# StanfordMSL/RATiLQR.jl

Hardware: AMD Instinct MI355X
Metric: iLEQG solves/sec (N=50, n=12, m=4) at CE batch=1024 (higher is better)
Workload: dtype f64

## Files before the change

ratilqr.jl_amd/csrc/driver.cpp:

```cpp
#include <hip/hip_runtime.h>

#include <algorithm>
#include <cctype>
#include <cmath>
#include <cstdint>
#include <cstdio>
#include <cstdlib>
#include <cstring>
#include <functional>
#include <initializer_list>
#include <string>
#include <vector>

#include "../../include/ratilqr.h"
#include "kernels.h"
#include "layout.h"
#include "wide.h"
#include "ce_device.h"
#include "policy_mc.h"
#include "rare_event.h"
#include "source_args.h"
#include "source_model.h"

static thread_local std::string g_err;
// ... 14 lines not shown
    int device = 0;
    hipStream_t stream = nullptr;
    hipStream_t stream2 = nullptr;
    hipEvent_t ev_a = nullptr, ev_b = nullptr;
    bool dual_forced = false;
    bool dual = false;
    bool speculate = false;
    bool fused = true;
    bool fused_req = true, rounds_only = false;
    int block_req = -1;
    bool wdiag = true;
    bool materialize = false;
    std::vector<double> x0_host, u0_host;
    int fused_occ2 = -1;
    bool fused_dual = true;
    int block_mode = -1;
    int block_max_b = 512;
    int n_cu = 256;
    long long *d_xw = nullptr;
    int *d_duo_count = nullptr;
    bool lq_replay = true;
    bool lq_replay_last = true;
    bool lq_replay_stack = true;
    RecDev rec = {};
    size_t rec_cap = 0;
    unsigned xepoch = 0;
    int *d_census = nullptr;
    bool block_shape = true;
    bool block_helpers = true;
    bool block_acl = false;
    int path_fixed = RAT_PATH_AUTO;
    bool fly_multi = true;
    bool fly = true;
    rat_ileqg_opts opts;
    OptsDev opd;
    int Bmax = 0, E = 1;
    bool have_problem = false;
    int n = 0, m = 0, N = 0;
    ProblemDev pb;
    bool wide = false;
    WideProblemDev wpb;
    double *w_xs = nullptr, *w_us = nullptr, *w_L = nullptr, *w_dl = nullptr;
    double *w_gq = nullptr, *w_gr = nullptr, *w_gc = nullptr;
    int *w_nom = nullptr, *w_hn = nullptr;
    std::vector<void *> pb_allocs, st_allocs;
    std::vector<double> hW;
// ... 183 lines not shown
    {"ce_device", [](rat_handle h, int64_t v) { h->ce_device = (v != 0); }, [](rat_handle h) -> int64_t { return h->ce_device; }},
    {"pets_device", [](rat_handle h, int64_t v) { h->pets_device = (v != 0); }, [](rat_handle h) -> int64_t { return h->pets_device; }},
    {"psweep", [](rat_handle h, int64_t v) { h->psweep = (v < 2) ? 0 : (int)std::min<int64_t>(v, 4); }, [](rat_handle h) -> int64_t { return h->psweep; }},
    {"psw_hop", [](rat_handle h, int64_t v) { h->psw_hop = (int)std::max<int64_t>(1, v); }, [](rat_handle h) -> int64_t { return h->psw_hop; }},
    {"psw_hop_e", [](rat_handle h, int64_t v) { h->psw_hop_e = (int)std::max<int64_t>(1, v); }, [](rat_handle h) -> int64_t { return h->psw_hop_e; }},
    {"spec_force", [](rat_handle h, int64_t v) { h->spec_force = (v != 0); }, [](rat_handle h) -> int64_t { return h->spec_force; }},
    {"spec_width", [](rat_handle, int64_t) {}, [](rat_handle h) -> int64_t { return h->E; }},
    {"block_psw", [](rat_handle h, int64_t v) { h->block_psw = (v != 0); }, [](rat_handle h) -> int64_t { return h->block_psw; }},
    {"psw_duo", [](rat_handle h, int64_t v) { h->psw_duo = (v != 0); }, [](rat_handle h) -> int64_t { return h->psw_duo; }},
    {"psw_prl", [](rat_handle h, int64_t v) { h->psw_prl = (v != 0); }, [](rat_handle h) -> int64_t { return h->psw_prl; }},
    {"prl_elem", [](rat_handle h, int64_t v) { h->prl_elem = (int)std::max<int64_t>(1, v); }, [](rat_handle h) -> int64_t { return h->prl_elem; }},
    {"prl_hop", [](rat_handle h, int64_t v) { h->prl_hop = (int)std::max<int64_t>(0, v); }, [](rat_handle h) -> int64_t { return h->prl_hop; }},
    {"prl_epi", [](rat_handle h, int64_t v) { h->prl_epi = (int)std::max<int64_t>(0, v); }, [](rat_handle h) -> int64_t { return h->prl_epi; }},
    {"prl_cuts", [](rat_handle, int64_t) {}, [](rat_handle h) -> int64_t { return h->prl_last; }},
    {"psw_duo_count", [](rat_handle h, int64_t) { if (h->d_duo_count) { (void)hipStreamSynchronize(h->stream); (void)hipMemset(h->d_duo_count, 0, sizeof(int)); } },
     [](rat_handle h) -> int64_t { int c = 0; if (h->d_duo_count) { (void)hipStreamSynchronize(h->stream); (void)hipMemcpy(&c, h->d_duo_count, sizeof(int), hipMemcpyDeviceToHost); } return c; }},
    {"lq_replay", [](rat_handle h, int64_t v) { h->lq_replay = (v != 0); }, [](rat_handle h) -> int64_t { return h->lq_replay; }},
    {"lq_replay_count", [](rat_handle h, int64_t) { if (h->rec.count) { (void)hipStreamSynchronize(h->stream); (void)hipMemset(h->rec.count, 0, sizeof(int)); } },
     [](rat_handle h) -> int64_t { int c = 0; if (h->rec.count) { (void)hipStreamSynchronize(h->stream); (void)hipMemcpy(&c, h->rec.count, sizeof(int), hipMemcpyDeviceToHost); } return c; }},
    {"lq_replay_last", [](rat_handle h, int64_t v) { h->lq_replay_last = (v != 0); }, [](rat_handle h) -> int64_t { return h->lq_replay_last; }},
    {"lq_replay_last_count", [](rat_handle h, int64_t) { if (h->rec.count) { (void)hipStreamSynchronize(h->stream); (void)hipMemset(h->rec.count + 1, 0, sizeof(int)); } },
     [](rat_handle h) -> int64_t { int c = 0; if (h->rec.count) { (void)hipStreamSynchronize(h->stream); (void)hipMemcpy(&c, h->rec.count + 1, sizeof(int), hipMemcpyDeviceToHost); } return c; }},
    {"lq_replay_stack", [](rat_handle h, int64_t v) { h->lq_replay_stack = (v != 0); }, [](rat_handle h) -> int64_t { return h->lq_replay_stack; }},
    {"psw_acl", [](rat_handle h, int64_t v) { h->psw_acl = (v != 0); }, [](rat_handle h) -> int64_t { return h->psw_acl; }},
    {"psw_comp", [](rat_handle h, int64_t v) { h->psw_comp = (int)std::max<int64_t>(100, v); }, [](rat_handle h) -> int64_t { return h->psw_comp; }},
    {"src_tpw", [](rat_handle h, int64_t v) { h->src_tpw = (v >= 64) ? 64 : (v >= 32 ? 32 : 16); }, [](rat_handle h) -> int64_t { return h->src_tpw; }},
    {"src_pets_tpw", [](rat_handle h, int64_t v) { h->src_pets_tpw = (v >= 64) ? 64 : (v >= 32 ? 32 : 16); }, [](rat_handle h) -> int64_t { return h->src_pets_tpw; }},
    {"mc_cost_K", [](rat_handle, int64_t) {}, [](rat_handle h) -> int64_t { return h->mc_cost_K; }},
    {"src_mc_tpw", [](rat_handle h, int64_t v) { h->src_mc_tpw = (v >= 64) ? 64 : (v >= 32 ? 32 : 16); }, [](rat_handle h) -> int64_t { return h->src_mc_tpw; }},
    {"tail_dense", [](rat_handle h, int64_t v) { h->tail_dense = (v != 0); }, [](rat_handle h) -> int64_t { return h->tail_dense; }},
    {"src_un_loads", [](rat_handle, int64_t) {}, [](rat_handle h) -> int64_t { return h->src_un_loads; }},
};
static void finish_switches(rat_handle h) {
    h->E = (h->spec_force || h->E_req < 1) ? std::max(h->E_req, 1) : 1;
    if (!h->dual_forced) h->dual = h->E > 1;
    h->fused = h->fused_req && !(h->speculate || h->dual || h->E != 1);
    h->block_mode = h->rounds_only ? 0 : h->block_req;
}
static void debug_from_env(rat_handle h) {
    for (const DebugSwitch &sw : debug_switches) {
        std::string name = "RATILQR_";
        for (const char *c = sw.key; *c; ++c) name += (char)toupper((unsigned char)*c);
        if (const char *e = getenv(name.c_str())) {
            char *end = nullptr;
            const long long v = strtoll(e, &end, 10);
            if (end != e) sw.set(h, (int64_t)v);
// ... 960 lines not shown
    if (path == PATH_ROUNDS) launch_init_state(st, h->opd, theta_dev, h->stream);
    RolloutArgs ra; ra.st = st; ra.pb = h->pb; ra.op = h->opd; ra.dump = h->d_dump; ra.mode = 0; ra.x0 = h->d_x0; ra.u0 = h->d_u0; ra.notile = 0; ra.multi = 0;
    if (path != PATH_ROUNDS) {
        FusedArgs fa;
        fa.sw = sweep_args(h, st, 0);
        fa.sw.prune = (h->prune && st.E > 1) ? 1 : 0;
        fa.ro = ra;
        fa.max_rounds = (int)std::min<int64_t>(((int64_t)h->opd.iter_max + 1) * 4002, 2000000000);
        fa.dual = h->fused_dual ? 1 : 0;
        fa.occ2 = (path == PATH_FUSED && h->fused_dual &&
                   (h->fused_occ2 > 0 ? B >= h->fused_occ2 : (h->fused_occ2 < 0 && h->pb.model == 1 && !h->materialize && B > 4 * (int64_t)h->n_cu))) ? 1 : 0;
        fa.mat = h->materialize ? 1 : 0;
        if (path == PATH_FUSED && h->lq_replay && fa.dual && !fa.occ2 && !fa.mat && h->pb.model == 1 && h->pb.kappa == 0.0 && h->pb.W_diag &&
            !h->pb.W_tv && !h->pb.cost_tv && st.N <= ROLLIN_NST) {
            const size_t need = (size_t)B * st.N * REC_STEP;
            if (need > h->rec_cap) {
                if (h->rec.m) { HIPCHK(hipStreamSynchronize(h->stream)); HIPCHK(hipFree(h->rec.m)); h->rec.m = nullptr; h->rec_cap = 0; }
                HIPCHK(hipMalloc((void **)&h->rec.m, need * sizeof(double)));
                h->rec_cap = need;
            }
            fa.sw.rec = h->rec;
            fa.sw.rec.last = h->lq_replay_last ? 1 : 0;
            fa.sw.rec.stack = h->lq_replay_stack ? 1 : 0;
        }
        fa.theta_in = theta_dev;
        fa.out_value = out.value; fa.out_status = out.status; fa.out_iters = out.iters; fa.out_ls = out.ls;
        fa.out_cost = out.cost; fa.kl_bound = out.kl_bound;
        fa.init_x = fa.init_u = fa.init_t = nullptr;
        fa.census = (h->block_shape && h->E == 1 && B <= 2 * h->n_cu) ? h->d_census : nullptr;
        fa.helpers = (fa.census && B <= h->n_cu && h->block_helpers) ? 1 : 0;
        fa.acl = h->block_acl ? 1 : 0;
        const bool psw = path == PATH_BLOCK && h->block_psw && fa.helpers && !h->materialize && solve_block_psw_supported(fa);
        fa.duo_stride = 0; fa.xepoch = 0; fa.xw = nullptr; fa.duo_count = nullptr;
        if (psw && h->psw_duo && 2 * ((B + 7) & ~7) <= h->n_cu) {
            fa.duo_stride = (B + 7) & ~7; fa.xepoch = ++h->xepoch; fa.xw = h->d_xw; fa.duo_count = h->d_duo_count;
        }
        const bool own_init = psw && h->init_lazy && !h->init_traj_valid && h->init_batches == 0;
        if (h->init_share && h->pb.model == 1 && st.N <= ROLLIN_NST && !own_init) {
            ensure_init_traj(h, ra, theta_dev);
            fa.init_x = h->d_init_x; fa.init_u = h->d_init_u; fa.init_t = h->d_init_t;
        }
        h->init_batches++;
        fa.prl = 0;
        h->prl_last = 0;
        if (psw) {
            fa.acl = (h->psw_acl || h->block_acl) ? 1 : 0;
// ... 2994 lines not shown
```

ratilqr.jl_amd/csrc/kernels.h:

```cpp
#pragma once
#include <hip/hip_runtime.h>

#include "layout.h"

#ifndef RAT_ROLLOUT_MFMA4
#define RAT_ROLLOUT_MFMA4 1
#endif

#define REC_STEP 256
struct RecDev {
    double *m;
    double *mu;
    double *rprod;
    int *rexp;
    int *gen;
    int *lgen;
    int *count;
    int last;
    int stack;
};

struct SweepArgs {
    StateDev st;
    ProblemDev pb;
    OptsDev op;
    int mode;
    int k_first;
    const double *dl_in;
    double mu_op;
    double *op_out;
    double *dump;
    int fly;
    int prune;
    RecDev rec;
};

#define PSW_MAXP 8
struct PswCuts { int P; int cut[PSW_MAXP + 2]; };

#define PRL_WAVES 4
struct PrlCuts { int cut[PRL_WAVES + 1]; };

// ... 106 lines not shown
```

ratilqr.jl_amd/csrc/kernels.hip:

```cpp
#include <hip/hip_runtime.h>
#include <math.h>

#include "layout.h"
#include "kernels.h"

#include "device_utils.h"
#include "rat_normal.h"
#include "rat_philox.h"
#include "rat_pow.h"
#include "sweep_dual.h"

#define PART_SWEEP 1
#define PART_ROLL 2
#define PART_FUSED 4
#define PART_BLOCK2 8
#define PART_BLOCK3 16
#define PART_BLOCK5 32
#define PART_BLOCK8 64
#define PART_MISC 128
#define PART_PSW 256
#define PART_BPSW 512
#define PART_BPSW1 1024
#ifndef RAT_PART
#define RAT_PART 2047
// ... 2160 lines not shown
__device__ __forceinline__ const FusedArgs &phase_args(const FusedArgs &fa) {
    if (!LOCAL) return fa;
    auto kp = (const __attribute__((address_space(4))) FusedArgs *)__builtin_amdgcn_kernarg_segment_ptr();
    asm volatile("" : "+s"(kp));
    return *(const FusedArgs *)kp;
}
template <bool LOCAL>
__device__ __forceinline__ RolloutArgs rollout_view(const FusedArgs &pa, const int mode) {
    RolloutArgs ra;
    if (!LOCAL) { ra = pa.ro; ra.mode = mode; return ra; }
    ra.st = pa.sw.st; ra.pb = pa.sw.pb; ra.op = pa.sw.op;
    ra.mode = mode; ra.x0 = pa.ro.x0; ra.u0 = pa.ro.u0; ra.dump = pa.ro.dump; ra.notile = pa.ro.notile; ra.multi = pa.ro.multi;
    return ra;
}

template <int MODEL, bool CTV, int WM, bool DUALF, bool STG, bool OCC2 = false, bool MAT = false, bool RPL = false>
__global__ __launch_bounds__(64, OCC2 ? 2 : 1) void solve_fused_kernel(FusedArgs fa) {
    const int b = blockIdx.x;
    const StateDev &st = fa.sw.st;
#ifdef RAT_DIAG_PHASES
    const unsigned long long dg_t0 = __builtin_readcyclecounter();
    int dg_pi = 0;
#endif
    __shared__ double wls[DUALF ? WLS_DUAL : WLS_SWEEP];
    __shared__ double shxu[16];
    __shared__ double stg[STG ? STG_DOUBLES : 1];
    constexpr int FLYF = (MODEL == 1 && ((DUALF && STG && !OCC2) || (OCC2 && !DUALF && !STG)) && !MAT) ? (CTV ? 2 : 1) : 0;
    constexpr bool NT = FLYF != 0;
    constexpr bool PL = (MODEL == 1);
    constexpr bool RM4 = RAT_ROLLOUT_MFMA4 && MODEL == 1 && STG && !OCC2;
    if (threadIdx.x == 0) {
        const FusedArgs &pa = phase_args<PL>(fa);
        init_state_body(pa.sw.st, pa.sw.op, pa.theta_in, b);
        if (RPL) { pa.sw.rec.gen[b] = 0; pa.sw.rec.lgen[2 * b] = 0; pa.sw.rec.lgen[2 * b + 1] = 0; }
    }
    PHASE_FENCE();
    {
        const FusedArgs &pi = phase_args<PL>(fa);
        if (NT && pi.init_x) {
            copy_initial(pi.sw.st, pi.init_x, pi.init_u, pi.init_t, b);
        } else {
            const RolloutArgs ra = rollout_view<PL>(pi, 0);
            rollin_body<MODEL, 0, CTV, STG, true, OCC2 ? OCC2_PREFETCH : ROLLIN_PREFETCH, NT>(ra, b, shxu, stg);
        }
        PHASE_MARK();
        PHASE_FENCE();
        PHASE_MARK();
        if (DUALF) {
            SweepArgs sa = phase_args<PL>(fa).sw; sa.mode = 6;
            sweep_dual_body<WM, false, FLYF, RPL>(sa, b, wls);
            PHASE_MARK();
            PHASE_FENCE();
            if (threadIdx.x == 0) commit_init_body(phase_args<PL>(fa).sw.st, b);
            PHASE_FENCE();
            PHASE_MARK();
        } else {
            SweepArgs sa = phase_args<PL>(fa).sw; sa.mode = 2;
            sweep_body<false, false, WM, false, OCC2 ? OCC2_SWZ : 0, FLYF>(sa, b, wls);
            PHASE_MARK();
            PHASE_FENCE();
            PHASE_MARK();
        }
    }
    for (int guard = 0; guard < fa.max_rounds; ++guard) {
        const int v_stat = __atomic_load_n(&st.status[b], __ATOMIC_RELAXED), v_act = __atomic_load_n(&st.ls_active[b], __ATOMIC_RELAXED);
        if (__builtin_amdgcn_readfirstlane(v_stat) != ST_RUNNING) break;
        if (!__builtin_amdgcn_readfirstlane(v_act)) {
            SweepArgs sa = phase_args<PL>(fa).sw; sa.mode = 0;
            sweep_body<true, false, WM, false, OCC2 ? OCC2_SWZ : 0, FLYF, false, RPL>(sa, b, wls);
            PHASE_MARK();
            PHASE_FENCE();
            PHASE_MARK();
            continue;
        }
        {
            const RolloutArgs ra = rollout_view<PL>(phase_args<PL>(fa), 1);
            rollin_body<MODEL, 1, CTV, STG, true, OCC2 ? OCC2_PREFETCH : ROLLIN_PREFETCH, NT, RM4>(ra, b, shxu, stg);
            PHASE_MARK();
            PHASE_FENCE();
            PHASE_MARK();
            bool pair = DUALF;
            if (DUALF) {
                const FusedArgs &pe = phase_args<PL>(fa);
                const double v_dc = *(const volatile double *)&pe.sw.st.d_c[b], v_mu = *(const volatile double *)&pe.sw.st.mu[b];
                const int v_it = __atomic_load_n(&pe.sw.st.iter[b], __ATOMIC_RELAXED);
                const double dc = readlane_f64(v_dc, 0), mu = readlane_f64(v_mu, 0);
                const bool ends = (pe.sw.op.d > dc && mu <= pe.sw.op.mu_min) || __builtin_amdgcn_readfirstlane(v_it) == pe.sw.op.iter_max;
                pair = !ends;
            }
            if (pair) {
                SweepArgs sa = phase_args<PL>(fa).sw; sa.mode = 7;
                if (!(RPL && replay_dual_body(sa, b, wls))) sweep_dual_body<WM, true, FLYF, RPL>(sa, b, wls);
            } else {
                SweepArgs sa = phase_args<PL>(fa).sw; sa.mode = 1;
                if (!(RPL && replay_eval_body(sa, b, wls))) sweep_body<false, false, WM, true, OCC2 ? OCC2_SWZ : 0, FLYF>(sa, b, wls);
            }
            PHASE_MARK();
            PHASE_FENCE();
            if (threadIdx.x == 0) { const FusedArgs &pa = phase_args<PL>(fa); ls_select_body(pa.sw.st, pa.sw.op, b, nullptr); }
            PHASE_FENCE();
            PHASE_MARK();
        }
    }
    PHASE_FENCE();
    if (threadIdx.x == 0) {
        const FusedArgs &pa = phase_args<PL>(fa);
        gather_body(pa.sw.st, b, pa.out_value, pa.out_status, pa.out_iters, pa.out_ls, pa.out_cost, pa.kl_bound);
    }
}


#if RAT_PART & PART_FUSED
void launch_solve_fused(const FusedArgs &fa, hipStream_t s) {
    const int B = fa.sw.st.B;
    if (B <= 0) return;
// ... 1158 lines not shown
```

ratilqr.jl_amd/csrc/layout.h:

```cpp
#pragma once

#define RAT_NP 12
#define RAT_MP 4
#define RAT_PD 16
#define RAT_AUG 12

#define TS_C34 256
#define TS_R5  352
#define TS_QR  400
#define TS_q   416
#define TS_PAD 418
#define TSTRIDE 420
#define TS_INFO 417
#define TT_Q   0
#define TT_QV  144
#define TT_q   156
#define TTERM  158
#define TT_INFO 157

#define TS_LIVE(l) (((l) & 15) < 12)
#define TS_CL(l) (((l) >> 4) * 12 + ((l) & 15))
#define TS_REG(R, l) ((R) < 2 ? 2 * (l) + (R) : (R) == 2 ? 128 + 2 * (l) : (R) == 6 ? 129 + 2 * (l) : \
                      (R) < 5 ? (TS_LIVE(l) ? TS_C34 + 2 * TS_CL(l) + ((R) - 3) : TS_PAD + ((R) - 3)) : \
                                (TS_LIVE(l) ? TS_R5 + TS_CL(l) : TS_PAD))
#define TS_ZPOS(i, c) TS_REG(((i) * 16 + (c)) >> 6, ((i) * 16 + (c)) & 63)
#define TS_CPOS(i, c) TS_REG(3 + (((i) * 16 + (c)) >> 6), ((i) * 16 + (c)) & 63)

#define XSTR 12
#define USTR 4
#define LSTR 48

#define DUMP_S   0
#define DUMP_SV  144
#define DUMP_s   156
#define DUMP_g   157
#define DUMP_G   161
#define DUMP_H   209
#define DUMP_STRIDE 225

#define WLS_SWEEP 232
#define WLS_DUAL  400
#define ROLLIN_NST 52
#define STG_CL ((ROLLIN_NST * LSTR + 63) / 64)
#define STG_CX (((ROLLIN_NST + 1) * XSTR + 63) / 64)
#define STG_CU ((ROLLIN_NST * USTR + 63) / 64)
#define STG_DOUBLES ((STG_CL + STG_CX + 2 * STG_CU) * 64)
#define STG_PAD (STG_CL * 64)

#define ST_RUNNING (-1)
#define CTR_RING 8

struct ProblemDev {
    int model, n, m, N, cost_tv, W_tv;
    int W_diag;
    const double *Zt;
    const double *Ctab;
    const double *lin;
    const double *q0;
    const double *Qf;
    const double *qvf;
    double q0f, kappa;
    double pl_a, pl_b, pl_p, pl_pu, pl_cx, pl_cu, pl_h;
    const double *Winv;
    const double *Wp;
    const double *epiv;
    const double *logdetW;
    const double *Wdg;
};

// ... 33 lines not shown
```

ratilqr.jl_amd/csrc/sweep_dual.h:

```cpp
#pragma once
#include "device_utils.h"
#include "kernels.h"
#include "layout.h"

struct FlyCtx {
    double zt[3], dg[3];
    d4 cc;
    double mq, kappa;
    const double *xh;
    const double *ctab;
};
__device__ __forceinline__ void fly_init(FlyCtx &fc, const ProblemDev &pb, const double *xh, int l, int g, int j, bool tv) {
    fc.mq = (j < 12) ? 1.0 : 0.0;
    fc.kappa = pb.kappa;
    fc.xh = xh;
    fc.ctab = pb.Ctab;
#pragma unroll
    for (int r = 0; r < 3; ++r) { fc.zt[r] = pb.Zt[64 * r + l]; fc.dg[r] = (j == 4 * r + g) ? 1.0 : 0.0; }
    fc.cc = (d4){0, 0, 0, 0};
    if (!tv) {
#pragma unroll
        for (int r = 0; r < 3; ++r) fc.cc[r] = pb.Ctab[64 * r + l] * fc.mq;
        fc.cc[3] = pb.Ctab[192 + l];
    }
// ... 23 lines not shown
__device__ __forceinline__ void dload(DTile &tr, const double *__restrict__ tp, int lx, int l, int j,
                                      const double *__restrict__ Lp, double mL, int g, const FlyCtx *fc = nullptr, int t = 0) {
    if (FLY) {
        tr.xj = fc->xh[(long)t * XSTR + ((j < 12) ? j : 11)];
        if (FLY == 2) {
            const double *__restrict__ C = fc->ctab + (long)t * 256;
#pragma unroll
            for (int r = 0; r < 4; ++r) tr.c[r] = C[64 * r + l];
        }
    } else {
        const double2 *__restrict__ t2 = reinterpret_cast<const double2 *>(tp);
        const int c34 = TS_REG(3, l), r5 = TS_REG(5, l);
        const double2 w0 = t2[l], w1 = t2[64 + l], w2 = *reinterpret_cast<const double2 *>(tp + c34);
        tr.z[0] = w0.x; tr.z[1] = w0.y; tr.z[2] = w1.x; tr.z[3] = 0.0;
        tr.c[0] = w2.x; tr.c[1] = w2.y; tr.c[2] = tp[r5];
        tr.c[3] = w1.y;
    }
    tr.x = tp[TS_QR + lx];
    const int jc = (j < 12) ? j : 11;
    tr.la = HASL ? Lp[g * 12 + jc] * mL : 0.0;
}

template <int WM, bool HASL, int FLY = 0, bool REC = false>
__device__ __forceinline__ void sweep_dual_body(const SweepArgs &a, const int b, double *const wls) {
    int lane_ = threadIdx.x & 63;
    asm volatile("" : "+v"(lane_));
    const int l_ = lane_, g_ = l_ >> 4, j_ = l_ & 15;
    const int l = l_, g = g_, j = j_;
    const StateDev &st = a.st;
    const ProblemDev &pb = a.pb;
    [[maybe_unused]] const int dgs = 20 + 4 * (a.mode - 6);
    BODY_MARK(a.dump, dgs + 0);
    int slot, cidx = -1;
    const int v_act = st.ls_active[b], v_flag = st.flag_c[b * st.E], v_nom = st.slot_nom[b], v_stat = st.status[b], v_sel = st.lsel[b];
    const int s_act = wave_uniform(v_act), s_flag = wave_uniform(v_flag), s_nom = wave_uniform(v_nom), s_stat = wave_uniform(v_stat), sel = wave_uniform(v_sel);
    const double theta = st.theta[b], muB = st.mu[b];
    if (a.mode == 7) {
        if (!s_act) return;
        cidx = b * st.E;
        if (s_flag == 2) return;
        slot = cand_slot(b, 0, s_nom, st.E);
    } else {
        if (s_stat != ST_RUNNING) return;
        slot = b * (st.E + 1) + s_nom;
    }
    const double muA = (a.mode == 6) ? 0.0 : muB;
    const int N = st.N;
// ... 44 lines not shown
    const double coef = (theta != 0.0) ? -1.0 / (2.0 * theta) : 0.0;

    d4 vA, vB;
    {
        const double *__restrict__ tt = tile0 + (long)N * TSTRIDE;
#pragma unroll
        for (int r = 0; r < 3; ++r) {
            const int i = 4 * r + g;
            const double te = tt[(j < 12) ? TT_Q + i * 12 + j : TT_QV + i];
            vA[r] = (j <= 12) ? te : 0.0;
        }
        const double t3 = tt[(j < 12) ? TT_QV + j : TT_q];
        vA[3] = (g == 0 && j <= 12) ? (j < 12 ? t3 : 2.0 * t3) : 0.0;
        vB = vA;
    }
#ifdef RAT_DIAG_PHASES
    if (a.mode == 7) { asm volatile("s_waitcnt vmcnt(0)" ::: "memory"); BODY_MARK(a.dump, 29); }
#endif
    double raccA = 0.0, raccB = 0.0, rprodA = 1.0, rprodB = 1.0;
    int rexpA = 0, rexpB = 0;
    int failA = 0, deadB = 0;
    [[maybe_unused]] double *const recp = REC ? a.rec.m + (long)b * N * REC_STEP + 4 * l : nullptr;
    [[maybe_unused]] double rchk = 0.0;

    DIAG_DECL
    auto step = [&](const int t, const DTile &cur) -> int {
        int l = l_, g = g_, j = j_;
        asm volatile("" : "+v"(l), "+v"(g), "+v"(j));
        DIAG_START();
        if (WM == 1) {
#pragma unroll
            for (int r = 0; r < 3; ++r) { winv[r] = pb.Winv[(long)t * 192 + 64 * r + l]; wp[r] = pb.Wp[(long)t * 192 + 64 * r + l]; }
            { const double *ept = pb.epiv + (long)t * 16; epall = ((((ept[0] * ept[2]) * ept[4]) * ept[6]) * ept[8]) * ept[10]; }
        }
        d4 cz, ccs;
        if (!FLY) { cz = cur.z; ccs = cur.c; }
        else {
#pragma unroll
            for (int r = 0; r < 3; ++r) cz[r] = fx_diag(fc.zt[r], fc.dg[r], fc.kappa, cur.xj);
            cz[3] = 0.0;
            if (FLY == 2) { ccs[0] = cur.c[0] * fc.mq; ccs[1] = cur.c[1] * fc.mq; ccs[2] = cur.c[2] * fc.mq; ccs[3] = cur.c[3]; }
            else ccs = fc.cc;
        }
        d4 xzA, xzB;
        if (WM != 2) {
            xzA = mm3(vA, cz, (d4){0, 0, 0, 0});
// ... 68 lines not shown
        const double fvA = tmA[3] + cur.x, fvB = tmB[3] + cur.x;
        exA[g * 16 + j] = ghA; exB[g * 16 + j] = ghB;
        exA[fbo] = fvA; exB[fbo] = fvB;
        if (HASL) lbufA[l] = cur.la;
        DIAG_STAMP(3, ghB);
        WAVE_SYNC();
        const double hA0 = exA[hoff[0]], hA1 = exA[hoff[1]], hA2 = exA[hoff[2]], hA3 = exA[hoff[3]];
        const double gaA = fma(ghA, m12, exA[gaoff]);
        const double uaA = HASL ? ua_entry(hA0, hA1, hA2, hA3, lbufA[j], lbufA[16 + j], lbufA[32 + j], lbufA[48 + j], gaA) : gaA;
        const double hB0 = exB[hoff[0]], hB1 = exB[hoff[1]], hB2 = exB[hoff[2]], hB3 = exB[hoff[3]];
        const double gaB = fma(ghB, m12, exB[gaoff]);
        const double h00 = exB[12], h01 = exB[13], h02 = exB[14], h03 = exB[15];
        const double h11 = exB[16 + 13], h12 = exB[16 + 14], h13 = exB[16 + 15];
        const double h22 = exB[32 + 14], h23 = exB[32 + 15], h33 = exB[48 + 15];
        const double g0 = exB[goff[0]], g1 = exB[goff[1]], g2 = exB[goff[2]], g3 = exB[goff[3]];
        const double d0 = h00, i0 = fast_rcp(d0);
        const double l10 = h01 * i0, l20 = h02 * i0, l30 = h03 * i0;
        const double d1 = h11 - l10 * h01, i1 = fast_rcp(d1);
        const double l21 = (h12 - l20 * h01) * i1, l31 = (h13 - l30 * h01) * i1;
        const double d2 = h22 - l20 * h02 - l21 * (l21 * d1), i2 = fast_rcp(d2);
        const double l32 = (h23 - l30 * h02 - l31 * (l21 * d1)) * i2;
        const double d3 = h33 - l30 * h03 - l31 * (l31 * d1) - l32 * (l32 * d2), i3 = fast_rcp(d3);
        if (!deadB && !(d0 > 0.0 && d1 > 0.0 && d2 > 0.0 && d3 > 0.0)) deadB = 1;
        const double y0 = -g0;
        const double y1 = -g1 - l10 * y0;
        const double y2 = -g2 - l20 * y0 - l21 * y1;
        const double y3 = -g3 - l30 * y0 - l31 * y1 - l32 * y2;
        const double x3 = y3 * i3;
        const double x2 = y2 * i2 - l32 * x3;
        const double x1 = y1 * i1 - l21 * x2 - l31 * x3;
        const double x0 = y0 * i0 - l10 * x1 - l20 * x2 - l30 * x3;
        const double laB = ((x0 * em.e0[0] + x1 * em.e1[0]) + x2 * em.e0[1]) + x3 * em.e1[1];
        const double uaB = ua_entry(hB0, hB1, hB2, hB3, x0, x1, x2, x3, gaB);
        pgl[(long)t * sgl] = (j <= 12) ? laB : 0.0;
        d4 fxA, fxB;
#pragma unroll
        for (int r = 0; r < 3; ++r) { fxA[r] = fma(fA[r], m12, exA[foff[r]]); fxB[r] = fma(fB[r], m12, exB[foff[r]]); }
        const double qc = readlane_f64(cur.x, 16);
        fxA[3] = fma(fvA, mA_, (2.0 * qc + vA[3]) * mB_);
        fxB[3] = fma(fvB, mA_, (2.0 * qc + vB[3]) * mB_);
        DIAG_STAMP(4, uaB);
        d4 vnB = MFMA(laB, uaB, fxB);
        vnB = MFMA(gaB, laB, vnB);
        if (HASL) {
            d4 vnA = MFMA(cur.la, uaA, fxA);
            vA = MFMA(gaA, cur.la, vnA);
// ... 12 lines not shown
    BODY_MARK(a.dump, dgs + 1);
    for (int t = N - 1; t >= 0; t -= 2) {
        {
            const int tn = (t > 0) ? t - 1 : 0;
            dload<HASL, FLY>(rb2, tile0 + (long)tn * TSTRIDE, lx, l, j, Lb + (long)tn * LSTR, mL, g, &fc, tn);
        }
        if (step(t, ra)) break;
        if (t == 0) break;
        {
            const int tn = (t > 1) ? t - 2 : 0;
            dload<HASL, FLY>(ra, tile0 + (long)tn * TSTRIDE, lx, l, j, Lb + (long)tn * LSTR, mL, g, &fc, tn);
        }
        if (step(t - 1, rb2)) break;
    }
    BODY_MARK(a.dump, dgs + 2);
#ifdef RAT_DIAG
    if (l_ == 0 && blockIdx.x < 8 && a.dump)
        for (int q = 0; q < 6; ++q) a.dump[128 + blockIdx.x * 8 + q] = (double)dg_acc[q];
#endif
    const double totA = sweep_scalars(wave_sum(raccA), coef, rprodA, rexpA, theta != 0.0);
    (void)raccB; (void)rprodB; (void)rexpB;
    if (REC) {
        const bool bad = failA || deadB || theta == 0.0 || __ballot(!(rchk == 0.0));
        if (l == 12) rec_close(a.rec, b, sel ^ 1, bad, muB, rprodB, rexpB);
    }
    if (l == 12) {
        const double s0 = 0.5 * vA[3] + totA;
        if (a.mode == 7) {
            st.value_c[cidx] = s0;
            st.flag_c[cidx] = failA ? 1 : 0;
            if (a.prune) {
                const double cur = st.value[b], eps = st.ls_eps[b];
                const bool take = !failA && (isapprox_default(s0, cur) || s0 < cur || eps * a.op.lambda < a.op.eps_min);
                __atomic_store_n(&st.acc0[b], take ? 1 : 0, __ATOMIC_RELAXED);
            }
        } else {
            st.value[b] = failA ? INFINITY : s0;
            if (failA) st.status[b] = 1;
        }
        st.mu_spec[b] = muB;
        st.delta_spec[b] = st.delta[b];
        st.spec_st[b] = (failA || deadB == 1) ? 0 : (deadB == 2 ? 2 : 1);
    }
    BODY_MARK(a.dump, dgs + 3);
}


struct RTile {
    double2 m01, m2h;
    double x, xj, la;
};

template <bool GAINB, bool STACK = false>
__device__ __forceinline__ bool replay_body(const SweepArgs &a, const int b, double *const wls) {
    int lane_ = threadIdx.x & 63;
    asm volatile("" : "+v"(lane_));
    const int l_ = lane_, g_ = l_ >> 4, j_ = l_ & 15;
    const int l = l_, g = g_, j = j_;
    const StateDev &st = a.st;
    const ProblemDev &pb = a.pb;
    const RecDev &rc = a.rec;
    const int v_act = st.ls_active[b], v_flag = st.flag_c[b * st.E], v_nom = st.slot_nom[b], v_sel = st.lsel[b];
    const int v_gen = rc.gen[b], v_lg0 = rc.lgen[2 * b], v_lg1 = rc.lgen[2 * b + 1];
    const double v_theta = st.theta[b], v_mu = st.mu[b], v_rmu = rc.mu[b], v_rprod = rc.rprod[b];
    const int v_rexp = rc.rexp[b];
    const int s_act = wave_uniform(v_act), s_flag = wave_uniform(v_flag), s_nom = wave_uniform(v_nom), sel = wave_uniform(v_sel);
    const int gen = wave_uniform(v_gen), lg = wave_uniform(sel ? v_lg1 : v_lg0);
    const double theta = readlane_f64(v_theta, 0), mu = readlane_f64(v_mu, 0), rmu = readlane_f64(v_rmu, 0);
    if (!s_act || s_flag == 2 || a.prune) return false;
    if (!GAINB && !rc.last) return false;
    if (gen <= 0 || lg != gen || theta == 0.0 || __double_as_longlong(mu) != 0 || __double_as_longlong(rmu) != 0) return false;
    const int slot = cand_slot(b, 0, s_nom, st.E);
    const int N = st.N;
    const double *__restrict__ tile0 = st.tiles + tile_slot(st, b, slot) * st.tile_stride;
    const double *__restrict__ xh = st.xs + (long)slot * st.x_stride;
    const double *__restrict__ rp = rc.m + (long)b * N * REC_STEP + 4 * l;
    const int osel = sel ^ 1;
// ... 1 lines not shown
    double *__restrict__ Lout = st.L + (long)osel * st.l_half + (long)b * N * LSTR;
    double *__restrict__ dlout = st.dl + (long)osel * st.dl_half + (long)b * N * USTR;

    double *const lbuf = wls;
    double *const exA = wls + 64, *const exB = wls + 64 + 168;
    if (l < 8) { exA[80 + l] = 0.0; exB[80 + l] = 0.0; }

    const double m12 = (j < 12) ? 1.0 : 0.0;
    const double nth12 = -theta * m12;
    const double mA_ = (g == 0 && j < 12) ? 1.0 : 0.0, mB_ = (g == 0 && j == 12) ? 1.0 : 0.0;
    [[maybe_unused]] const double e00 = (g == 0) ? 1.0 : 0.0, e10 = (g == 1) ? 1.0 : 0.0, e01 = (g == 2) ? 1.0 : 0.0, e11 = (g == 3) ? 1.0 : 0.0;
    int hoff[4], foff[3];
    [[maybe_unused]] int goff[4];
#pragma unroll
    for (int k = 0; k < 4; ++k) {
        hoff[k] = (g <= k) ? (g * 16 + 12 + k) : (k * 16 + 12 + g);
        goff[k] = (j < 12) ? (k * 16 + j) : (j == 12 ? 64 + 12 + k : 80);
    }
#pragma unroll
    for (int r = 0; r < 3; ++r) foff[r] = (j == 12) ? (64 + 4 * r + g) : 80;
    const int gaoff = (j == 12) ? (64 + 12 + g) : 80;
    const int lx = (l < 17) ? l : TS_PAD - TS_QR;
    const int jc = (j < 12) ? j : 11;
    const int svo = (g == 0) ? 84 + j : 104 + l, fbo = (g == 0) ? 64 + j : 104 + l;
    [[maybe_unused]] double *const pgl = (j < 12) ? Lout + g * 12 + j : (j == 12 ? dlout + g : sample_sink(st, b) + l);
    [[maybe_unused]] const long sgl = (j < 12) ? LSTR : (j == 12 ? USTR : 0);
    double zt[3], dg[3], nwrow[3];
#pragma unroll
    for (int r = 0; r < 3; ++r) { zt[r] = pb.Zt[64 * r + l]; dg[r] = (j == 4 * r + g) ? 1.0 : 0.0; nwrow[r] = -pb.Wdg[4 * r + g]; }
    const double kappa = pb.kappa;
    const double coef = -1.0 / (2.0 * theta);

    d4 vA, vB;
    {
        const double *__restrict__ tt = tile0 + (long)N * TSTRIDE;
#pragma unroll
        for (int r = 0; r < 3; ++r) {
            const int i = 4 * r + g;
            const double te = tt[(j < 12) ? TT_Q + i * 12 + j : TT_QV + i];
            vA[r] = (j <= 12) ? te : 0.0;
        }
        const double t3 = tt[(j < 12) ? TT_QV + j : TT_q];
        vA[3] = (g == 0 && j <= 12) ? (j < 12 ? t3 : 2.0 * t3) : 0.0;
        vB = vA;
    }
    double raccA = 0.0;

    auto load = [&](RTile &tr, const int t) {
        const double2 *__restrict__ q = reinterpret_cast<const double2 *>(rp + (long)t * REC_STEP);
        tr.m01 = q[0];
        tr.m2h = q[1];
        tr.x = tile0[(long)t * TSTRIDE + TS_QR + lx];
        tr.xj = xh[(long)t * XSTR + jc];
        tr.la = Lb[(long)t * LSTR + g * 12 + jc] * m12;
    };
    auto step = [&](const int t, const RTile &cur) -> bool {
        int l = l_, g = g_, j = j_;
        asm volatile("" : "+v"(l), "+v"(g), "+v"(j));
        d4 cz;
#pragma unroll
        for (int r = 0; r < 3; ++r) cz[r] = fx_diag(zt[r], dg[r], kappa, cur.xj);
        cz[3] = 0.0;
        double probe = (cz[0] + cz[1]) + cz[2];
        probe += (vA[0] + vA[1]) + (vA[2] + vA[3]);
        if (GAINB) probe += (vB[0] + vB[1]) + (vB[2] + vB[3]);
        if (__ballot(!(probe - probe == 0.0))) return false;
        const double m0 = cur.m01.x, m1 = cur.m01.y, m2 = cur.m2h.x, gh = cur.m2h.y;
        exA[svo] = vA[3];
        if (GAINB) exB[svo] = vB[3];
        raccA = racc_diag(raccA, nth12, exA[84 + j], m0, m1, m2, exA[84 + g], exA[84 + 4 + g], exA[84 + 8 + g]);
        d4 mw;
        mw[0] = m0 * nwrow[0]; mw[1] = m1 * nwrow[1]; mw[2] = m2 * nwrow[2]; mw[3] = 0.0;
        const d4 y2 = mm3(mw, cz, (d4){0, 0, 0, 0});
        double tA12, tB12 = 0.0;
        if (GAINB && STACK) {
            d4 vS;
#pragma unroll
            for (int r = 0; r < 3; ++r) vS[r] = row_ror8_merge<0x2>(vA[r], vB[r]);
            vS[3] = 0.0;
            const d4 tm = mm3(vS, y2, (d4){0, 0, 0, 0});
            tA12 = tm[3];
            tB12 = tm[1];
        } else {
            const d4 tmA = mm3(vA, y2, (d4){0, 0, 0, 0});
            tA12 = tmA[3];
            if (GAINB) { const d4 tmB = mm3(vB, y2, (d4){0, 0, 0, 0}); tB12 = tmB[3]; }
        }
        const double fvA = tA12 + cur.x, fvB = tB12 + cur.x;
        exB[g * 16 + j] = gh;
        exA[fbo] = fvA;
        lbuf[l] = cur.la;
        if (GAINB) exB[fbo] = fvB;
        WAVE_SYNC();
        const double h0 = exB[hoff[0]], h1 = exB[hoff[1]], h2 = exB[hoff[2]], h3 = exB[hoff[3]];
        const double qc = readlane_f64(cur.x, 16);
        if (GAINB) {
            const double gaB = fma(gh, m12, exB[gaoff]);
            const double h00 = exB[12], h01 = exB[13], h02 = exB[14], h03 = exB[15];
            const double h11 = exB[16 + 13], h12 = exB[16 + 14], h13 = exB[16 + 15];
            const double h22 = exB[32 + 14], h23 = exB[32 + 15], h33 = exB[48 + 15];
            const double g0 = exB[goff[0]], g1 = exB[goff[1]], g2 = exB[goff[2]], g3 = exB[goff[3]];
            const double d0 = h00, i0 = fast_rcp(d0);
            const double l10 = h01 * i0, l20 = h02 * i0, l30 = h03 * i0;
            const double d1 = h11 - l10 * h01, i1 = fast_rcp(d1);
            const double l21 = (h12 - l20 * h01) * i1, l31 = (h13 - l30 * h01) * i1;
            const double d2 = h22 - l20 * h02 - l21 * (l21 * d1), i2 = fast_rcp(d2);
            const double l32 = (h23 - l30 * h02 - l31 * (l21 * d1)) * i2;
            const double d3 = h33 - l30 * h03 - l31 * (l31 * d1) - l32 * (l32 * d2), i3 = fast_rcp(d3);
            const double y0 = -g0;
            const double y1 = -g1 - l10 * y0;
            const double yy2 = -g2 - l20 * y0 - l21 * y1;
            const double y3 = -g3 - l30 * y0 - l31 * y1 - l32 * yy2;
            const double x3 = y3 * i3;
            const double x2 = yy2 * i2 - l32 * x3;
            const double x1 = y1 * i1 - l21 * x2 - l31 * x3;
            const double x0 = y0 * i0 - l10 * x1 - l20 * x2 - l30 * x3;
            const double laB = ((x0 * e00 + x1 * e10) + x2 * e01) + x3 * e11;
            const double uaB = ua_entry(h0, h1, h2, h3, x0, x1, x2, x3, gaB);
            pgl[(long)t * sgl] = (j <= 12) ? laB : 0.0;
            d4 fxB;
#pragma unroll
            for (int r = 0; r < 3; ++r) fxB[r] = exB[foff[r]];
            fxB[3] = fma(fvB, mA_, (2.0 * qc + vB[3]) * mB_);
            const d4 vn = MFMA(laB, uaB, fxB);
            vB = MFMA(gaB, laB, vn);
        }
        {
            const double gaA = fma(gh, m12, exA[gaoff]);
            const double uaA = ua_entry(h0, h1, h2, h3, lbuf[j], lbuf[16 + j], lbuf[32 + j], lbuf[48 + j], gaA);
            d4 fxA;
#pragma unroll
            for (int r = 0; r < 3; ++r) fxA[r] = exA[foff[r]];
            fxA[3] = fma(fvA, mA_, (2.0 * qc + vA[3]) * mB_);
            const d4 vn = MFMA(cur.la, uaA, fxA);
            vA = MFMA(gaA, cur.la, vn);
        }
        WAVE_SYNC();
        return true;
    };

    RTile r0, r1, r2;
    load(r0, N - 1);
    load(r1, (N > 1) ? N - 2 : 0);
    bool ok = true;
    for (int t = N - 1; t >= 0; t -= 3) {
        load(r2, (t > 1) ? t - 2 : 0);
        if (!step(t, r0)) { ok = false; break; }
        if (t == 0) break;
        load(r0, (t > 2) ? t - 3 : 0);
        if (!step(t - 1, r1)) { ok = false; break; }
        if (t == 1) break;
        load(r1, (t > 3) ? t - 4 : 0);
        if (!step(t - 2, r2)) { ok = false; break; }
    }
    WAVE_SYNC();
    if (!ok) return false;
    const double totA = sweep_scalars(wave_sum(raccA), coef, readlane_f64(v_rprod, 0), __builtin_amdgcn_readfirstlane(v_rexp), true);
    if (l == 12) {
        st.value_c[b * st.E] = 0.5 * vA[3] + totA;
        st.flag_c[b * st.E] = 0;
        if (GAINB) {
            st.mu_spec[b] = mu;
            st.delta_spec[b] = st.delta[b];
            st.spec_st[b] = 1;
            rc.lgen[2 * b + osel] = gen;
        }
    }
    if (l == 0) atomicAdd(rc.count + (GAINB ? 0 : 1), GAINB ? 2 : 1);
    return true;
}
__device__ __forceinline__ bool replay_dual_body(const SweepArgs &a, const int b, double *const wls) {
    return a.rec.stack ? replay_body<true, true>(a, b, wls) : replay_body<true>(a, b, wls);
}
__device__ __forceinline__ bool replay_eval_body(const SweepArgs &a, const int b, double *const wls) { return replay_body<false>(a, b, wls); }
```

Baseline: 4.032 million.

## Cache 4x4 LDL factors in LDS during dual sweep for replay reuse

During the recorded dual sweep, the per-step 4x4 LDL factor reciprocals and multipliers for branch B are written to a new LDS region, and a mark flag records whether the sweep was clean. When the LQ replay path later runs with gain B, it reads these cached factors instead of recomputing the factorization from the Hessian entries. It also hoists the per-step state-dependent finiteness probe into a single upfront check over the whole state trajectory, and drops the xj load from each tile. This costs more shared memory per block and adds LDS writes in the sweep, and the cached factors are only valid if the mark flag is kept in sync.

```diff
diff --git a/ratilqr.jl_amd/csrc/driver.cpp b/ratilqr.jl_amd/csrc/driver.cpp
--- a/ratilqr.jl_amd/csrc/driver.cpp
+++ b/ratilqr.jl_amd/csrc/driver.cpp
@@ -60,6 +60,7 @@
     bool lq_replay = true;
     bool lq_replay_last = true;
     bool lq_replay_stack = true;
+    bool lq_replay_ldsfac = true;
     RecDev rec = {};
     size_t rec_cap = 0;
     unsigned xepoch = 0;
@@ -289,6 +290,7 @@
     {"lq_replay_last_count", [](rat_handle h, int64_t) { if (h->rec.count) { (void)hipStreamSynchronize(h->stream); (void)hipMemset(h->rec.count + 1, 0, sizeof(int)); } },
      [](rat_handle h) -> int64_t { int c = 0; if (h->rec.count) { (void)hipStreamSynchronize(h->stream); (void)hipMemcpy(&c, h->rec.count + 1, sizeof(int), hipMemcpyDeviceToHost); } return c; }},
     {"lq_replay_stack", [](rat_handle h, int64_t v) { h->lq_replay_stack = (v != 0); }, [](rat_handle h) -> int64_t { return h->lq_replay_stack; }},
+    {"lq_replay_ldsfac", [](rat_handle h, int64_t v) { h->lq_replay_ldsfac = (v != 0); }, [](rat_handle h) -> int64_t { return h->lq_replay_ldsfac; }},
     {"psw_acl", [](rat_handle h, int64_t v) { h->psw_acl = (v != 0); }, [](rat_handle h) -> int64_t { return h->psw_acl; }},
     {"psw_comp", [](rat_handle h, int64_t v) { h->psw_comp = (int)std::max<int64_t>(100, v); }, [](rat_handle h) -> int64_t { return h->psw_comp; }},
     {"src_tpw", [](rat_handle h, int64_t v) { h->src_tpw = (v >= 64) ? 64 : (v >= 32 ? 32 : 16); }, [](rat_handle h) -> int64_t { return h->src_tpw; }},
@@ -1295,6 +1297,7 @@
             fa.sw.rec = h->rec;
             fa.sw.rec.last = h->lq_replay_last ? 1 : 0;
             fa.sw.rec.stack = h->lq_replay_stack ? 1 : 0;
+            fa.sw.rec.ldsfac = h->lq_replay_ldsfac ? 1 : 0;
         }
         fa.theta_in = theta_dev;
         fa.out_value = out.value; fa.out_status = out.status; fa.out_iters = out.iters; fa.out_ls = out.ls;
diff --git a/ratilqr.jl_amd/csrc/kernels.h b/ratilqr.jl_amd/csrc/kernels.h
--- a/ratilqr.jl_amd/csrc/kernels.h
+++ b/ratilqr.jl_amd/csrc/kernels.h
@@ -17,7 +17,8 @@
     int *lgen;
     int *count;
     int last;
-    int stack;
+    short stack;
+    short ldsfac;
 };
 
 struct SweepArgs {
diff --git a/ratilqr.jl_amd/csrc/kernels.hip b/ratilqr.jl_amd/csrc/kernels.hip
--- a/ratilqr.jl_amd/csrc/kernels.hip
+++ b/ratilqr.jl_amd/csrc/kernels.hip
@@ -2206,7 +2206,8 @@
     const unsigned long long dg_t0 = __builtin_readcyclecounter();
     int dg_pi = 0;
 #endif
-    __shared__ double wls[DUALF ? WLS_DUAL : WLS_SWEEP];
+    __shared__ alignas(RPL ? 16 : 8) double wls[(DUALF ? WLS_DUAL : WLS_SWEEP) + (RPL ? FAC_DOUBLES : 0)];
+    double *const fac = RPL ? wls + WLS_DUAL : nullptr;
     __shared__ double shxu[16];
     __shared__ double stg[STG ? STG_DOUBLES : 1];
     constexpr int FLYF = (MODEL == 1 && ((DUALF && STG && !OCC2) || (OCC2 && !DUALF && !STG)) && !MAT) ? (CTV ? 2 : 1) : 0;
@@ -2216,7 +2217,10 @@
     if (threadIdx.x == 0) {
         const FusedArgs &pa = phase_args<PL>(fa);
         init_state_body(pa.sw.st, pa.sw.op, pa.theta_in, b);
-        if (RPL) { pa.sw.rec.gen[b] = 0; pa.sw.rec.lgen[2 * b] = 0; pa.sw.rec.lgen[2 * b + 1] = 0; }
+        if (RPL) {
+            pa.sw.rec.gen[b] = 0; pa.sw.rec.lgen[2 * b] = 0; pa.sw.rec.lgen[2 * b + 1] = 0;
+            *reinterpret_cast<int *>(fac + FAC_MARK) = 0;
+        }
     }
     PHASE_FENCE();
     {
@@ -2232,7 +2236,7 @@
         PHASE_MARK();
         if (DUALF) {
             SweepArgs sa = phase_args<PL>(fa).sw; sa.mode = 6;
-            sweep_dual_body<WM, false, FLYF, RPL>(sa, b, wls);
+            sweep_dual_body<WM, false, FLYF, RPL>(sa, b, wls, fac);
             PHASE_MARK();
             PHASE_FENCE();
             if (threadIdx.x == 0) commit_init_body(phase_args<PL>(fa).sw.st, b);
@@ -2274,7 +2278,7 @@
             }
             if (pair) {
                 SweepArgs sa = phase_args<PL>(fa).sw; sa.mode = 7;
-                if (!(RPL && replay_dual_body(sa, b, wls))) sweep_dual_body<WM, true, FLYF, RPL>(sa, b, wls);
+                if (!(RPL && replay_dual_body(sa, b, wls, fac))) sweep_dual_body<WM, true, FLYF, RPL>(sa, b, wls, fac);
             } else {
                 SweepArgs sa = phase_args<PL>(fa).sw; sa.mode = 1;
                 if (!(RPL && replay_eval_body(sa, b, wls))) sweep_body<false, false, WM, true, OCC2 ? OCC2_SWZ : 0, FLYF>(sa, b, wls);
diff --git a/ratilqr.jl_amd/csrc/layout.h b/ratilqr.jl_amd/csrc/layout.h
--- a/ratilqr.jl_amd/csrc/layout.h
+++ b/ratilqr.jl_amd/csrc/layout.h
@@ -45,6 +45,11 @@
 #define STG_CX (((ROLLIN_NST + 1) * XSTR + 63) / 64)
 #define STG_CU ((ROLLIN_NST * USTR + 63) / 64)
 #define STG_DOUBLES ((STG_CL + STG_CX + 2 * STG_CU) * 64)
+#define FAC_STEP 10
+#define FAC_DUMP (FAC_STEP * ROLLIN_NST)
+#define FAC_MARK (FAC_DUMP + 2 * 64 + FAC_STEP - 2)
+#define FAC_DOUBLES (FAC_MARK + 2)
+#define XPROBE_N ((ROLLIN_NST * XSTR + 63) / 64)
 #define STG_PAD (STG_CL * 64)
 
 #define ST_RUNNING (-1)
diff --git a/ratilqr.jl_amd/csrc/sweep_dual.h b/ratilqr.jl_amd/csrc/sweep_dual.h
--- a/ratilqr.jl_amd/csrc/sweep_dual.h
+++ b/ratilqr.jl_amd/csrc/sweep_dual.h
@@ -69,7 +69,7 @@
 }
 
 template <int WM, bool HASL, int FLY = 0, bool REC = false>
-__device__ __forceinline__ void sweep_dual_body(const SweepArgs &a, const int b, double *const wls) {
+__device__ __forceinline__ void sweep_dual_body(const SweepArgs &a, const int b, double *const wls, double *const fac = nullptr) {
     int lane_ = threadIdx.x & 63;
     asm volatile("" : "+v"(lane_));
     const int l_ = lane_, g_ = l_ >> 4, j_ = l_ & 15;
@@ -160,6 +160,8 @@
     int failA = 0, deadB = 0;
     [[maybe_unused]] double *const recp = REC ? a.rec.m + (long)b * N * REC_STEP + 4 * l : nullptr;
     [[maybe_unused]] double rchk = 0.0;
+    [[maybe_unused]] double *const facp = REC ? fac + ((l == 0) ? 0 : FAC_DUMP + 2 * l) : nullptr;
+    [[maybe_unused]] const int facs = (l == 0) ? FAC_STEP : 0;
 
     DIAG_DECL
     auto step = [&](const int t, const DTile &cur) -> int {
@@ -274,6 +276,11 @@
         const double l32 = (h23 - l30 * h02 - l31 * (l21 * d1)) * i2;
         const double d3 = h33 - l30 * h03 - l31 * (l31 * d1) - l32 * (l32 * d2), i3 = fast_rcp(d3);
         if (!deadB && !(d0 > 0.0 && d1 > 0.0 && d2 > 0.0 && d3 > 0.0)) deadB = 1;
+        if (REC) {
+            double2 *const fq = reinterpret_cast<double2 *>(facp + t * facs);
+            fq[0] = make_double2(i0, i1); fq[1] = make_double2(i2, i3);
+            fq[2] = make_double2(l10, l20); fq[3] = make_double2(l30, l21); fq[4] = make_double2(l31, l32);
+        }
         const double y0 = -g0;
         const double y1 = -g1 - l10 * y0;
         const double y2 = -g2 - l20 * y0 - l21 * y1;
@@ -332,7 +339,10 @@
     (void)raccB; (void)rprodB; (void)rexpB;
     if (REC) {
         const bool bad = failA || deadB || theta == 0.0 || __ballot(!(rchk == 0.0));
-        if (l == 12) rec_close(a.rec, b, sel ^ 1, bad, muB, rprodB, rexpB);
+        if (l == 12) {
+            rec_close(a.rec, b, sel ^ 1, bad, muB, rprodB, rexpB);
+            *reinterpret_cast<int *>(fac + FAC_MARK) = bad ? 0 : 1;
+        }
     }
     if (l == 12) {
         const double s0 = 0.5 * vA[3] + totA;
@@ -358,11 +368,11 @@
 
 struct RTile {
     double2 m01, m2h;
-    double x, xj, la;
+    double x, la;
 };
 
-template <bool GAINB, bool STACK = false>
-__device__ __forceinline__ bool replay_body(const SweepArgs &a, const int b, double *const wls) {
+template <bool GAINB, bool STACK = false, bool LDSF = false>
+__device__ __forceinline__ bool replay_body(const SweepArgs &a, const int b, double *const wls, [[maybe_unused]] const double *const fac = nullptr) {
     int lane_ = threadIdx.x & 63;
     asm volatile("" : "+v"(lane_));
     const int l_ = lane_, g_ = l_ >> 4, j_ = l_ & 15;
@@ -410,14 +420,20 @@
     const int gaoff = (j == 12) ? (64 + 12 + g) : 80;
     const int lx = (l < 17) ? l : TS_PAD - TS_QR;
     const int jc = (j < 12) ? j : 11;
+    double xp[XPROBE_N];
+#pragma unroll
+    for (int k = 0; k < XPROBE_N; ++k) { const int i = 64 * k + l; xp[k] = xh[(i < N * XSTR) ? i : 0]; }
     const int svo = (g == 0) ? 84 + j : 104 + l, fbo = (g == 0) ? 64 + j : 104 + l;
     [[maybe_unused]] double *const pgl = (j < 12) ? Lout + g * 12 + j : (j == 12 ? dlout + g : sample_sink(st, b) + l);
     [[maybe_unused]] const long sgl = (j < 12) ? LSTR : (j == 12 ? USTR : 0);
     double zt[3], dg[3], nwrow[3];
 #pragma unroll
     for (int r = 0; r < 3; ++r) { zt[r] = pb.Zt[64 * r + l]; dg[r] = (j == 4 * r + g) ? 1.0 : 0.0; nwrow[r] = -pb.Wdg[4 * r + g]; }
-    const double kappa = pb.kappa;
     const double coef = -1.0 / (2.0 * theta);
+    d4 cz;
+#pragma unroll
+    for (int r = 0; r < 3; ++r) cz[r] = fx_diag(zt[r], dg[r], pb.kappa, 0.0);
+    cz[3] = 0.0;
 
     d4 vA, vB;
     {
@@ -439,20 +455,19 @@
         tr.m01 = q[0];
         tr.m2h = q[1];
         tr.x = tile0[(long)t * TSTRIDE + TS_QR + lx];
-        tr.xj = xh[(long)t * XSTR + jc];
         tr.la = Lb[(long)t * LSTR + g * 12 + jc] * m12;
     };
     auto step = [&](const int t, const RTile &cur) -> bool {
         int l = l_, g = g_, j = j_;
         asm volatile("" : "+v"(l), "+v"(g), "+v"(j));
-        d4 cz;
-#pragma unroll
-        for (int r = 0; r < 3; ++r) cz[r] = fx_diag(zt[r], dg[r], kappa, cur.xj);
-        cz[3] = 0.0;
-        double probe = (cz[0] + cz[1]) + cz[2];
-        probe += (vA[0] + vA[1]) + (vA[2] + vA[3]);
+        double probe = (vA[0] + vA[1]) + (vA[2] + vA[3]);
         if (GAINB) probe += (vB[0] + vB[1]) + (vB[2] + vB[3]);
         if (__ballot(!(probe - probe == 0.0))) return false;
+        [[maybe_unused]] double2 f01, f23, f45, f67, f89;
+        if (GAINB && LDSF) {
+            const double2 *const fq = reinterpret_cast<const double2 *>(fac + t * FAC_STEP);
+            f01 = fq[0]; f23 = fq[1]; f45 = fq[2]; f67 = fq[3]; f89 = fq[4];
+        }
         const double m0 = cur.m01.x, m1 = cur.m01.y, m2 = cur.m2h.x, gh = cur.m2h.y;
         exA[svo] = vA[3];
         if (GAINB) exB[svo] = vB[3];
@@ -484,17 +499,27 @@
         const double qc = readlane_f64(cur.x, 16);
         if (GAINB) {
             const double gaB = fma(gh, m12, exB[gaoff]);
-            const double h00 = exB[12], h01 = exB[13], h02 = exB[14], h03 = exB[15];
-            const double h11 = exB[16 + 13], h12 = exB[16 + 14], h13 = exB[16 + 15];
-            const double h22 = exB[32 + 14], h23 = exB[32 + 15], h33 = exB[48 + 15];
             const double g0 = exB[goff[0]], g1 = exB[goff[1]], g2 = exB[goff[2]], g3 = exB[goff[3]];
-            const double d0 = h00, i0 = fast_rcp(d0);
-            const double l10 = h01 * i0, l20 = h02 * i0, l30 = h03 * i0;
-            const double d1 = h11 - l10 * h01, i1 = fast_rcp(d1);
-            const double l21 = (h12 - l20 * h01) * i1, l31 = (h13 - l30 * h01) * i1;
-            const double d2 = h22 - l20 * h02 - l21 * (l21 * d1), i2 = fast_rcp(d2);
-            const double l32 = (h23 - l30 * h02 - l31 * (l21 * d1)) * i2;
-            const double d3 = h33 - l30 * h03 - l31 * (l31 * d1) - l32 * (l32 * d2), i3 = fast_rcp(d3);
+            double i0, i1, i2, i3, l10, l20, l30, l21, l31, l32;
+            if (LDSF) {
+                i0 = f01.x; i1 = f01.y; i2 = f23.x; i3 = f23.y;
+                l10 = f45.x; l20 = f45.y; l30 = f67.x; l21 = f67.y; l31 = f89.x; l32 = f89.y;
+            } else {
+                const double h00 = exB[12], h01 = exB[13], h02 = exB[14], h03 = exB[15];
+                const double h11 = exB[16 + 13], h12 = exB[16 + 14], h13 = exB[16 + 15];
+                const double h22 = exB[32 + 14], h23 = exB[32 + 15], h33 = exB[48 + 15];
+                const double d0 = h00;
+                i0 = fast_rcp(d0);
+                l10 = h01 * i0; l20 = h02 * i0; l30 = h03 * i0;
+                const double d1 = h11 - l10 * h01;
+                i1 = fast_rcp(d1);
+                l21 = (h12 - l20 * h01) * i1; l31 = (h13 - l30 * h01) * i1;
+                const double d2 = h22 - l20 * h02 - l21 * (l21 * d1);
+                i2 = fast_rcp(d2);
+                l32 = (h23 - l30 * h02 - l31 * (l21 * d1)) * i2;
+                const double d3 = h33 - l30 * h03 - l31 * (l31 * d1) - l32 * (l32 * d2);
+                i3 = fast_rcp(d3);
+            }
             const double y0 = -g0;
             const double y1 = -g1 - l10 * y0;
             const double yy2 = -g2 - l20 * y0 - l21 * y1;
@@ -530,6 +555,12 @@
     RTile r0, r1, r2;
     load(r0, N - 1);
     load(r1, (N > 1) ? N - 2 : 0);
+    {
+        double xprobe = 0.0;
+#pragma unroll
+        for (int k = 0; k < XPROBE_N; ++k) xprobe = fma(xp[k] * xp[k], 0.0, xprobe);
+        if (__ballot(!(xprobe == 0.0))) return false;
+    }
     bool ok = true;
     for (int t = N - 1; t >= 0; t -= 3) {
         load(r2, (t > 1) ? t - 2 : 0);
@@ -557,7 +588,9 @@
     if (l == 0) atomicAdd(rc.count + (GAINB ? 0 : 1), GAINB ? 2 : 1);
     return true;
 }
-__device__ __forceinline__ bool replay_dual_body(const SweepArgs &a, const int b, double *const wls) {
+__device__ __forceinline__ bool replay_dual_body(const SweepArgs &a, const int b, double *const wls, const double *const fac = nullptr) {
+    const bool ldsf = fac && a.rec.ldsfac && wave_uniform(*reinterpret_cast<const int *>(fac + FAC_MARK)) != 0;
+    if (ldsf) return a.rec.stack ? replay_body<true, true, true>(a, b, wls, fac) : replay_body<true, false, true>(a, b, wls, fac);
     return a.rec.stack ? replay_body<true, true>(a, b, wls) : replay_body<true>(a, b, wls);
 }
 __device__ __forceinline__ bool replay_eval_body(const SweepArgs &a, const int b, double *const wls) { return replay_body<false>(a, b, wls); }
```

Result: no change. 4.064 million, median of 6 (+0.8%).
